# willi-menapace/PlayableEnvironments

Hardware: AMD Instinct MI355X
Metric: Mrays/s (higher is better)
Workload: dtype f32; 1 GPU; tennis renderer, 256x256 frame per GPU (rank r renders the frame of seed 1234 + r), 4 objects, 64+128 hierarchical samples/ray (coarse+fine networks), eval - BASELINE.json configs[1]; rays_per_gpu=65536, frames_per_gpu=1, parallelism=frame shard x1

## Files before the change

### include/playrender.h

```cpp
#ifndef PLAYRENDER_H
#define PLAYRENDER_H

#include <stddef.h>
#include <stdint.h>

#ifdef __cplusplus
extern "C" {
#endif

#define PR_ABI_VERSION 5
#define PR_MAX_OBJECTS 8
#define PR_MAX_LAYERS 12
#define PR_MAX_OCTAVES 16

typedef enum pr_status {
    PR_OK = 0,
    PR_ERR_INVALID = -1,
    PR_ERR_WORKSPACE = -2,
    PR_ERR_HIP = -3,
    PR_ERR_NO_DEVICE = -4
} pr_status;

#define PR_FLAG_PERTURB        1u
#define PR_FLAG_CANONICAL_POSE 2u
#define PR_FLAG_FIX_OVERLAPS   4u
#define PR_FLAG_NAIVE_MLP      8u
#define PR_FLAG_TRAIN_BN       16u

#define PR_FLAG_SAVE_FOR_BACKWARD 32u

#define PR_FLAG_GATE_HEAD 64u

#define PR_FLAG_DEVICE_NOISE 128u

#define PR_FLAG_SIGMOID_FEATURES 512u
#define PR_FLAG_SPLIT_BACKWARD 1024u
#define PR_FLAG_DIVERGENCE_GRAD 256u

typedef struct pr_linear_t {
    const float* weight;
    const float* bias;
    int32_t out_features;
    int32_t in_features;
} pr_linear_t;

typedef struct pr_object_model_t {
    int32_t kind;
    int32_t has_bender;
    int32_t positions;
    int32_t style_features;
    int32_t deformation_features;
    int32_t output_features;
    int32_t layers_width;
    int32_t backbone_count;
    int32_t skip_layer_idx;
    int32_t octaves;
    int32_t bender_width;
    int32_t bender_count;
    int32_t bender_skip;
// ... 246 lines not shown
```

### playableenvironments_amd/_lib.py

```python
from __future__ import annotations

import ctypes as C
import os
from typing import Optional

PR_MAX_OBJECTS = 8
PR_MAX_LAYERS = 12
PR_MAX_OCTAVES = 16

PR_FLAG_PERTURB = 1
PR_FLAG_CANONICAL_POSE = 2
PR_FLAG_FIX_OVERLAPS = 4
PR_FLAG_NAIVE_MLP = 8
PR_FLAG_TRAIN_BN = 16
PR_FLAG_SAVE_FOR_BACKWARD = 32
PR_FLAG_GATE_HEAD = 64
PR_FLAG_DEVICE_NOISE = 128
PR_FLAG_DIVERGENCE_GRAD = 256
PR_FLAG_SIGMOID_FEATURES = 512
PR_FLAG_SPLIT_BACKWARD = 1024
PR_PRECISION_FP32 = 0
PR_PRECISION_F16X3 = 1
PR_PRECISION_F16 = 2
PR_PROFILE_CATEGORIES = 8

c_float_p = C.POINTER(C.c_float)
c_int32_p = C.POINTER(C.c_int32)
c_uint8_p = C.POINTER(C.c_uint8)


class Linear(C.Structure):
    _fields_ = [("weight", C.c_void_p), ("bias", C.c_void_p), ("out_features", C.c_int32), ("in_features", C.c_int32)]


class ObjectModel(C.Structure):
    _fields_ = [
        ("kind", C.c_int32), ("has_bender", C.c_int32), ("positions", C.c_int32),
        ("style_features", C.c_int32), ("deformation_features", C.c_int32), ("output_features", C.c_int32),
        ("layers_width", C.c_int32), ("backbone_count", C.c_int32), ("skip_layer_idx", C.c_int32),
        ("octaves", C.c_int32), ("bender_width", C.c_int32), ("bender_count", C.c_int32),
        ("bender_skip", C.c_int32), ("bender_octaves", C.c_int32),
        ("bender_octave_weights", C.c_float * PR_MAX_OCTAVES),
        ("bbox", C.c_float * 6),
# ... 188 lines not shown
```

### playableenvironments_amd/csrc/backward.hip

```cpp
#include "pr_common.h"

#include <algorithm>
#include <map>
#include <utility>
#include <mutex>
#include "composite_dev.h"

namespace pr {

constexpr int BWD_SPLITS = 128;
constexpr int MAX_FCHUNK_B = 4;

struct CompositeBwdObject {
    const float* t;
    const float* sigma;
    const int32_t* slot;
    const float* dispmag;
    const float* feat;
    NoiseRef noise;
    int positions;
    pr_entry_grads_t g;
    float* g_feat;
    float* g_sigma;
    float* g_t;
    float* g_dm;
    const float* g_sample_t;
    const float* divergence;
    float* g_div;
// ... 1277 lines not shown
            gp.g_enc[k] = gtake(sizeof(float) * cap * encp);
            gp.gsr4[k] = gtake(sizeof(float) * cap * 4);
            gp.g_x[k] = gtake(sizeof(float) * cap * 3);
            gp.g_in6[k] = gtake(sizeof(float) * cap * 6);
            if (bc) {
                gp.g_braw4[k] = gtake(sizeof(float) * cap * 4);
                gp.bgstack[k] = gtake(sizeof(float) * cap * BWp * (size_t)bc);
                gp.g_benc[k] = gtake(sizeof(float) * cap * binp);
            }
        }
        gp.tn_partial_floats = tn_floats;
        gp.tn_partial = gtake(sizeof(float) * tn_floats);
        gp.zero_begin = goff;
        for (int k = 0; k < c.objects; ++k) {
            gp.sums[k] = gtake(sizeof(double) * 4 * MAX_WIDTH);
            gp.tables[k] = gtake(sizeof(float) * (size_t)c.frames * 4 * MAX_WIDTH);
        }
        gp.counters = gtake(sizeof(int32_t) * (4 * PR_MAX_OBJECTS + 8 * 4));
        gp.zero_bytes = goff - gp.zero_begin;
        gp.end = goff;
        gp.usable = !(c.flags & PR_FLAG_DIVERGENCE_GRAD) && (goff - lane_begin) <= GROUP_SCRATCH_LIMIT;
        if (gp.usable) bp->bytes = goff;
    }
    return PR_OK;
}

static int lane_stream(hipStream_t caller, hipStream_t* out) {
    static std::mutex mu;
    static std::map<std::pair<int, hipStream_t>, hipStream_t> streams;
    int dev = 0;
    PR_CHECK_HIP(hipGetDevice(&dev));
    std::lock_guard<std::mutex> lock(mu);
    hipStream_t& slot = streams[std::make_pair(dev, caller)];
    if (!slot) PR_CHECK_HIP(hipStreamCreateWithFlags(&slot, hipStreamNonBlocking));
    *out = slot;
    return PR_OK;
}

static int stream_wait(hipStream_t waiter, hipStream_t on) {
    constexpr int RING = 8;
    struct Ring { hipEvent_t e[RING] = {}; int next = 0; };
    static thread_local std::map<int, Ring> rings;
    int dev = 0;
    PR_CHECK_HIP(hipGetDevice(&dev));
    Ring& ring = rings[dev];
    hipEvent_t& e = ring.e[ring.next];
    ring.next = (ring.next + 1) % RING;
    if (!e) PR_CHECK_HIP(hipEventCreateWithFlags(&e, hipEventDisableTiming));
    PR_CHECK_HIP(hipEventRecord(e, on));
    PR_CHECK_HIP(hipStreamWaitEvent(waiter, e, 0));
    return PR_OK;
}

struct GemmCtx {
    const int32_t* rows;
    int max_rows;
    float* partial;
    hipStream_t s;
    float* gstack;
    float* chain_packed;
    size_t cap;
    const float* dw_acts;
    size_t dw_stride;
    const float* dw_in0;
};

static int weight_grad(const GemmCtx& g, const float* dY, int ldy, int n_out, const float* X, int ldx, int n_in, float* dW,
                       int ldw, float* dbias) {
    if (!dW && !dbias) return PR_OK;
    GemmTN p;
    memset(&p, 0, sizeof(p));
    p.A = dY; p.lda = ldy; p.B = X; p.ldb = ldx;
    p.rows = g.rows; p.ni = n_out; p.nj = n_in; p.splits = BWD_SPLITS;
// ... 928 lines not shown
```

### playableenvironments_amd/csrc/composite.hip

```cpp
#include "pr_common.h"
#include "composite_dev.h"

namespace pr {

struct CompositeSmem {
    float* tt;
    float* sg;
    float* dm;
    float* wo;
    float* wg;
    float* al;
    float* dv;
    int* sl;
    unsigned int* key;
};

constexpr int MAX_FCHUNK = 4;

__device__ __forceinline__ void transmittance_weights(float* al, int n, int lane) {
    float carry = 1.0f;
    for (int base = 0; base < n; base += 64) {
        const int j = base + lane;
        const float a = (j < n) ? al[j] : 0.f;
        float incl = (j < n) ? __fadd_rn(__fsub_rn(1.0f, a), 1e-10f) : 1.0f;
#pragma unroll
        for (int d = 1; d < 64; d <<= 1) {
            const float o = __shfl_up(incl, d, 64);
            if (lane >= d) incl *= o;
        }
        float excl = __shfl_up(incl, 1, 64);
        if (lane == 0) excl = 1.0f;
        if (j < n) al[j] = a * (carry * excl);
        carry *= __shfl(incl, 63, 64);
    }
}

constexpr int ROWS_IN_FLIGHT = 8;

__device__ __forceinline__ float sigmoid_of(float x) { return 1.0f / (1.0f + expf(-x)); }

template <int CW>
__device__ __forceinline__ void transmittance_weights_block(float* al, int n, float* totals, int wave, int lane) {
    if (CW == 1) {
        transmittance_weights(al, n, lane);
        return;
    }
    const int seg = (((n + CW - 1) / CW) + 63) & ~63;
    const int begin = wave * seg;
    const int end = (begin + seg < n) ? begin + seg : n;
    float carry = 1.0f;
    for (int base = begin; base < end; base += 64) {
        const int j = base + lane;
        const float a = (j < end) ? al[j] : 0.f;
        float incl = (j < end) ? __fadd_rn(__fsub_rn(1.0f, a), 1e-10f) : 1.0f;
#pragma unroll
        for (int d = 1; d < 64; d <<= 1) {
            const float o = __shfl_up(incl, d, 64);
            if (lane >= d) incl *= o;
        }
        float excl = __shfl_up(incl, 1, 64);
// ... 2 lines not shown
        carry *= __shfl(incl, 63, 64);
    }
    if (lane == 0) totals[wave] = carry;
    __syncthreads();
    float before = 1.0f;
    for (int w = 0; w < wave; ++w) before *= totals[w];
    if (wave > 0)
        for (int j = begin + lane; j < end; j += 64) al[j] *= before;
    __syncthreads();
}

template <int CW>
__device__ __forceinline__ float block_sum(float v, float* scratch, int wave, int lane) {
    v = wave_sum(v);
    if (CW == 1) return v;
    __syncthreads();
    if (lane == 0) scratch[wave] = v;
    __syncthreads();
    float total = 0.f;
    for (int w = 0; w < CW; ++w) total += scratch[w];
    return total;
}

template <int CW>
__global__ __launch_bounds__(64 * CW) void k_composite(CompositeParams p) {
    extern __shared__ __attribute__((aligned(16))) char raw_smem[];
    constexpr int CT = 64 * CW;
    const int S = p.sort_size;
    CompositeSmem sm;
    const int A = (p.total_positions + 63) & ~63;
    sm.key = reinterpret_cast<unsigned int*>(raw_smem);
    sm.tt = reinterpret_cast<float*>(sm.key + S);
    sm.sg = sm.tt + A;
    sm.dm = sm.sg + A;
    sm.wo = sm.dm + A;
    sm.wg = sm.sg;
    sm.al = sm.wo + A;
    const bool use_div = p.any_divergence != 0;
    sm.dv = use_div ? sm.al + A : nullptr;
    sm.sl = reinterpret_cast<int*>(sm.al + (use_div ? 2 * A : A));
    float* scratch = reinterpret_cast<float*>(sm.sl + A);
    unsigned long long* wide = p.fix_overlaps ? reinterpret_cast<unsigned long long*>(scratch + 4 * 64) : nullptr;

    const int tid = threadIdx.x, lane = tid & 63;
    const int wave = (CW == 1) ? 0 : __builtin_amdgcn_readfirstlane(tid >> 6);
    const long g = blockIdx.x;
    const float* d = p.ray_directions + (size_t)g * 3;
    const float norm = sqrtf(__fadd_rn(__fadd_rn(__fmul_rn(d[0], d[0]), __fmul_rn(d[1], d[1])), __fmul_rn(d[2], d[2])));
    const int PT = p.total_positions;

    {
        int off = 0;
        for (int k = 0; k < p.objects; ++k) {
            const CompositeObject& o = p.obj[k];
            const int P = o.positions;
            const size_t base = (size_t)g * P;
            for (int i = tid; i < P; i += CT) {
                sm.tt[off + i] = o.t[base + i];
                sm.sg[off + i] = o.sigma[base + i];
                sm.sl[off + i] = o.slot[base + i];
                sm.dm[off + i] = o.dispmag ? o.dispmag[base + i] : 0.f;
// ... 164 lines not shown
                w2 = sm.wg[off + i];
                take = row >= 0 && (w1 != 0.f || w2 != 0.f);
                if (p.sigmoid && row < 0) {
                    bare1 += w1;
                    bare2 += w2;
                }
            }
            const unsigned long long m = __ballot(take);
            if (take) {
                const int pos = off + begin + count + __popcll(m & ((1ull << lane) - 1ull));
                lrow[pos] = row;
                lw1[pos] = w1;
                sm.al[pos] = w2;
            }
            count += __popcll(m);
        }
        const int* rows_w = lrow + off + begin;
        const float* w1_w = lw1 + off + begin;
        const float* w2_w = sm.al + off + begin;
        float acco[MAX_FCHUNK];
#pragma unroll
        for (int c = 0; c < MAX_FCHUNK; ++c) acco[c] = 0.f;
        int i = 0;
        for (; i + ROWS_IN_FLIGHT <= count; i += ROWS_IN_FLIGHT) {
            float v[ROWS_IN_FLIGHT][MAX_FCHUNK];
#pragma unroll
            for (int u = 0; u < ROWS_IN_FLIGHT; ++u) {
                const float* f = o.feat + (size_t)rows_w[i + u] * F;
#pragma unroll
                for (int c = 0; c < MAX_FCHUNK; ++c) {
                    const int ch = lane + 64 * c;
                    v[u][c] = (ch < F) ? f[ch] : 0.f;
                    if (p.sigmoid) v[u][c] = sigmoid_of(v[u][c]);
                }
            }
#pragma unroll
            for (int u = 0; u < ROWS_IN_FLIGHT; ++u) {
                const float w1 = w1_w[i + u], w2 = w2_w[i + u];
#pragma unroll
                for (int c = 0; c < MAX_FCHUNK; ++c) {
                    acco[c] = __fadd_rn(acco[c], __fmul_rn(w1, v[u][c]));
                    accg[c] = __fadd_rn(accg[c], __fmul_rn(w2, v[u][c]));
                }
            }
        }
        for (; i < count; ++i) {
            const float* f = o.feat + (size_t)rows_w[i] * F;
            const float w1 = w1_w[i], w2 = w2_w[i];
#pragma unroll
            for (int c = 0; c < MAX_FCHUNK; ++c) {
                const int ch = lane + 64 * c;
                float v = (ch < F) ? f[ch] : 0.f;
                if (p.sigmoid) v = sigmoid_of(v);
                acco[c] = __fadd_rn(acco[c], __fmul_rn(w1, v));
                accg[c] = __fadd_rn(accg[c], __fmul_rn(w2, v));
            }
        }
        if (p.sigmoid) {
            bare1 = wave_sum(bare1);
            bare2 = wave_sum(bare2);
// ... 54 lines not shown
                scratch[wave * 64 + lane] = accg[c];
                __syncthreads();
                if (wave == 0)
                    for (int w = 1; w < CW; ++w) accg[c] = __fadd_rn(accg[c], scratch[w * 64 + lane]);
            }
        }
        if (wave == 0) {
            const int frame = (int)(g / p.rays);
            int r = (int)(g - (long)frame * p.rays);
            int grp = 0;
            while (grp < p.decoder.groups - 1 && r >= p.decoder.rays[grp]) r -= p.decoder.rays[grp++];
            const int c0 = p.decoder.channel_begin[grp], c1 = p.decoder.channel_end[grp];
            const size_t cells = (size_t)p.decoder.rays[grp];
            float* map = p.decoder.map[grp] + (size_t)frame * (c1 - c0) * cells + r;
#pragma unroll
            for (int c = 0; c < MAX_FCHUNK; ++c) {
                const int ch = lane + 64 * c;
                if (ch >= c0 && ch < c1 && ch < F) map[(size_t)(ch - c0) * cells] = accg[c];
            }
        }
    }
}

int launch_composite(const CompositeParams& p, hipStream_t s) {
    PR_REQUIRE(p.F <= 64 * MAX_FCHUNK, "output_features %d exceeds %d", p.F, 64 * MAX_FCHUNK);
    PR_REQUIRE(p.sort_size >= p.total_positions && (p.sort_size & (p.sort_size - 1)) == 0, "bad sort size");
    for (int k = 0; k < p.objects; ++k)
        PR_REQUIRE(p.obj[k].positions <= 64 * 32, "positions per ray %d too large for the overlap mask", p.obj[k].positions);
    const size_t lds = (size_t)p.sort_size * 4 + (size_t)((p.total_positions + 63) & ~63) * (p.any_divergence ? 7 : 6) * 4 +
                       sizeof(float) * 4 * 64 + (p.fix_overlaps ? (size_t)p.sort_size * 8 : 0);
    PR_REQUIRE(lds <= 156 * 1024, "too many samples per ray for the compositing kernel (%d)", p.total_positions);
    if (p.decoder.groups > 0) {
        PR_REQUIRE(p.decoder.groups <= PR_MAX_DECODER_GROUPS, "decoder layout: %d groups (max %d)", p.decoder.groups, PR_MAX_DECODER_GROUPS);
        long sum = 0;
        for (int i = 0; i < p.decoder.groups; ++i) {
            PR_REQUIRE(p.decoder.rays[i] > 0 && p.decoder.width[i] > 0 && p.decoder.rays[i] % p.decoder.width[i] == 0,
                       "decoder layout: group %d has %d rays in rows of %d", i, p.decoder.rays[i], p.decoder.width[i]);
            PR_REQUIRE(p.decoder.channel_begin[i] >= 0 && p.decoder.channel_begin[i] < p.decoder.channel_end[i] && p.decoder.channel_end[i] <= p.F,
                       "decoder layout: group %d channel range [%d, %d) outside 0..%d", i, p.decoder.channel_begin[i], p.decoder.channel_end[i], p.F);
            PR_REQUIRE(p.decoder.map[i] != nullptr, "decoder layout: group %d has no map", i);
            sum += p.decoder.rays[i];
        }
        PR_REQUIRE(sum == p.rays, "decoder layout: the groups hold %ld rays, the call has %d", sum, p.rays);
    }
    const long total = (long)p.frames * p.rays;
    ProfileScope scope(1, s);
    if (p.total_positions >= 256) {
        PR_TRY(prepare_kernel(reinterpret_cast<const void*>(&k_composite<4>), 156 * 1024, nullptr));
        hipLaunchKernelGGL(k_composite<4>, dim3((unsigned)total), dim3(256), lds, s, p);
    } else {
        PR_TRY(prepare_kernel(reinterpret_cast<const void*>(&k_composite<1>), 156 * 1024, nullptr));
        hipLaunchKernelGGL(k_composite<1>, dim3((unsigned)total), dim3(64), lds, s, p);
    }
    PR_LAUNCH_CHECK();
    return PR_OK;
}

}
```

### playableenvironments_amd/csrc/pr_common.h

```cpp
#pragma once

#include <hip/hip_runtime.h>
#include <stdint.h>
#include <stdio.h>
#include <string.h>

#include "playrender.h"

namespace pr {

void set_error(const char* fmt, ...);

#define PR_CHECK_HIP(expr)                                                              \
    do {                                                                                \
        hipError_t _e = (expr);                                                         \
        if (_e != hipSuccess) {                                                         \
            pr::set_error("%s failed: %s (%s:%d)", #expr, hipGetErrorString(_e), __FILE__, __LINE__); \
            return PR_ERR_HIP;                                                          \
        }                                                                               \
    } while (0)

#define PR_REQUIRE(cond, ...)                                                           \
    do {                                                                                \
        if (!(cond)) {                                                                  \
// ... 344 lines not shown
    const float* t;
    const float* sigma;
    const int32_t* slot;
    const float* divergence;
    const float* dispmag;
    const float* feat;
    NoiseRef noise;
    int positions;
    pr_entry_t out;
};
struct CompositeParams {
    int frames, rays, objects, static_objects, F;
    int fix_overlaps;
    int any_divergence;
    int sigmoid;
    int total_positions;
    int sort_size;
    const float* ray_directions;
    NoiseRef noise_global;
    CompositeObject obj[PR_MAX_OBJECTS];
    pr_entry_t global;
    pr_decoder_layout_t decoder;
};
int launch_composite(const CompositeParams& p, hipStream_t s);

#define PR_TRY(expr)                 \
    do {                             \
        int _r = (expr);             \
        if (_r != PR_OK) return _r;  \
    } while (0)

struct SavedPlan {
    size_t rec_pos, rec_flat, row_flags, enc, act, h1, h2, batch, stat_count, bin, bact, braw, delta, div, bits, bbits, stats;
};
struct TypePlan {
    size_t t[PR_MAX_OBJECTS], sigma[PR_MAX_OBJECTS], slot[PR_MAX_OBJECTS], dispmag[PR_MAX_OBJECTS];
    size_t adain[PR_MAX_OBJECTS];
    size_t feat[PR_MAX_OBJECTS];
    int positions[PR_MAX_OBJECTS];
    size_t totals;
    size_t head_counts;
    size_t zero_begin, zero_bytes;
    SavedPlan saved[PR_MAX_OBJECTS];
};
struct Plan {
    TypePlan type[2];
    size_t block_sums, block_offsets;
    size_t rec_pos, rec_flat;
    size_t pend_act, pend_meta;
    size_t h1, h2, row_flags, stats, stat_count, batch_stats;
    size_t div_t0, div_ta, div_tb;
    size_t rec_pos_k[PR_MAX_OBJECTS], rec_flat_k[PR_MAX_OBJECTS];
    size_t bytes;
    int nblocks256;
};
int prepare_kernel(const void* kernel, int lds_bytes, int* cu_count);
int launch_zero_fill(void* dst, size_t bytes, hipStream_t s);
int validate_call(const pr_call_t& c, const pr_object_t* objs);
bool group_active(const pr_call_t& c);
bool group_train_active(const pr_call_t& c);
bool gate_active(const pr_call_t& c);
bool group_active(const pr_call_t& c);
int make_plan(const pr_call_t& c, const pr_object_t* objs, Plan* plan);
void bbox_split(const pr_object_model_t& m, float* lo, float* hi, float* size);
int build_mlp_layers(const pr_object_model_t& m, const ModelDims& d, const PackedLayout& l, const float* base,
                     MlpParams* p, bool split3 = false);

struct GemmNN {
    const float* A; int lda;
    const float* B; int ldb;
    float* C; int ldc;
    const int32_t* rows;
    int n, k;
    int accumulate;
    const float* mask; int ldm;
    int b_transposed;
    int k_valid;
};
int launch_gemm_nn(const GemmNN& p, int max_rows, hipStream_t s);

struct GemmTN {
    const float* A; int lda;
    const float* B; int ldb;
    float* C; int ldc;
// ... 84 lines not shown
    int32_t* counters;
    int split_precision;
};
size_t tn_all_partial_floats(int ni, int nj, long max_rows);
int launch_gemm_tn_all(TnAll& g, const long* max_rows, hipStream_t s);

struct DivergenceParams {
    const int32_t* total; int max_rows;
    const int32_t* rec_flat; const int32_t* row_flags; const float* rec_pos;
    NoiseRef noise;
    int positions;
    const float* bin; int bin_pad, benc, b_octaves;
    const float* bacts; size_t bact_stride; int BW, BWpad, b_count, b_skip, bin_real;
    const pr_linear_t* layers; pr_linear_t out_head;
    const float* braw;
    float lo[3], hi[3];
    int canonical;
    float* t0; float* ta; float* tb;
    float* tstack; size_t tstride;
    float* div;
};
int launch_divergence(const DivergenceParams& p, hipStream_t s);

struct ProfileScope {
    ProfileScope(int category, hipStream_t s);
    ~ProfileScope();
    int category_;
    hipStream_t stream_;
    hipEvent_t start_;
    bool active_;
};

#ifdef __HIPCC__
__device__ __forceinline__ void philox4x32_10(unsigned int c0, unsigned int c1, unsigned int c2, unsigned int c3, unsigned int k0,
                                              unsigned int k1, unsigned int* out) {
#pragma unroll
    for (int round = 0; round < 10; ++round) {
        const unsigned int hi0 = __umulhi(0xD2511F53u, c0), lo0 = 0xD2511F53u * c0;
        const unsigned int hi1 = __umulhi(0xCD9E8D57u, c2), lo1 = 0xCD9E8D57u * c2;
        const unsigned int n0 = hi1 ^ c1 ^ k0, n2 = hi0 ^ c3 ^ k1;
        c0 = n0; c1 = lo1; c2 = n2; c3 = lo0;
        k0 += 0x9E3779B9u;
        k1 += 0xBB67AE85u;
    }
    out[0] = c0; out[1] = c1; out[2] = c2; out[3] = c3;
}
// ... 74 lines not shown
```

### playableenvironments_amd/csrc/render.hip

```cpp
#include "pr_common.h"

#include <stdarg.h>

#include <atomic>
#include <mutex>
#include <vector>

namespace pr {

struct ProfileRecord { int category; hipEvent_t start, stop; };
static std::atomic<bool> g_profile_on{false};
static std::vector<ProfileRecord> g_profile;
static std::mutex g_profile_mutex;

int prepare_kernel(const void* kernel, int lds_bytes, int* cu_count) {
    struct Entry { const void* kernel; int device; int cus; };
    static std::vector<Entry> done;
    static std::mutex guard;
    int dev = 0;
    PR_CHECK_HIP(hipGetDevice(&dev));
    std::lock_guard<std::mutex> lock(guard);
    for (const Entry& e : done)
        if (e.kernel == kernel && e.device == dev) {
            if (cu_count) *cu_count = e.cus;
            return PR_OK;
        }
    PR_CHECK_HIP(hipFuncSetAttribute(kernel, hipFuncAttributeMaxDynamicSharedMemorySize, lds_bytes));
    hipDeviceProp_t prop;
// ... 37 lines not shown
    if (!active_) return;
    hipEvent_t stop;
    if (hipEventCreate(&stop) != hipSuccess) return;
    if (hipEventRecord(stop, stream_) != hipSuccess) {
        (void)hipEventDestroy(stop);
        (void)hipEventDestroy(start_);
        return;
    }
    std::lock_guard<std::mutex> lock(g_profile_mutex);
    g_profile.push_back(ProfileRecord{category_, start_, stop});
}

static thread_local char g_error[512] = "";

void set_error(const char* fmt, ...) {
    va_list ap;
    va_start(ap, fmt);
    vsnprintf(g_error, sizeof(g_error), fmt, ap);
    va_end(ap);
}

int build_mlp_layers(const pr_object_model_t& m, const ModelDims& d, const PackedLayout& l, const float* base,
                     MlpParams* p, bool split3);

static size_t align_up(size_t v) { return (v + 255) & ~(size_t)255; }

int validate_call(const pr_call_t& c, const pr_object_t* objs) {
    PR_REQUIRE(c.frames > 0 && c.rays > 0, "empty call: %d frames x %d rays", c.frames, c.rays);
    PR_REQUIRE(c.objects >= 1 && c.objects <= PR_MAX_OBJECTS, "objects %d out of range 1..%d", c.objects, PR_MAX_OBJECTS);
    PR_REQUIRE(c.static_objects >= 0 && c.static_objects <= c.objects, "static_objects %d out of range", c.static_objects);
    PR_REQUIRE((long)c.frames * c.rays < (1L << 31), "too many rays in one call");
    PR_REQUIRE(c.ray_origins && c.ray_directions && c.w2o && c.style && c.deformation && c.object_in_scene,
               "NULL input pointer");
    PR_REQUIRE(c.precision == PR_PRECISION_FP32 || c.precision == PR_PRECISION_F16X3 || c.precision == PR_PRECISION_F16,
               "unknown precision %d", c.precision);
    PR_REQUIRE(!(c.precision != PR_PRECISION_FP32 && (c.flags & PR_FLAG_TRAIN_BN)),
               "the fp16 kernels have no train-mode BatchNorm phases: use PR_PRECISION_FP32 for training");
    PR_REQUIRE(!(c.precision != PR_PRECISION_FP32 && (c.flags & PR_FLAG_SAVE_FOR_BACKWARD)),
               "differentiable calls run on the exact kernel: use PR_PRECISION_FP32 with PR_FLAG_SAVE_FOR_BACKWARD");
    PR_REQUIRE(!(c.flags & PR_FLAG_SAVE_FOR_BACKWARD) || !(c.flags & PR_FLAG_NAIVE_MLP), "the scalar debugging kernel saves nothing");
    for (int k = 0; k < c.objects; ++k) {
        const pr_object_model_t& m = objs[k].coarse;
        PR_REQUIRE(m.positions >= 1, "object %d: positions_count_coarse %d", k, m.positions);
        PR_REQUIRE(c.linspace_coarse[k] != nullptr, "object %d: linspace_coarse missing", k);
        PR_REQUIRE(objs[k].packed_coarse != nullptr, "object %d: packed coarse weights missing", k);
        PR_REQUIRE((long)c.frames * c.rays * (long)m.positions < (1L << 31), "too many samples in one call");
// ... 120 lines not shown
    if (div_t) {
        plan->div_t0 = take(sizeof(float) * div_t0);
        plan->div_ta = take(sizeof(float) * div_t);
        plan->div_tb = take(sizeof(float) * div_t);
    }
    if (c.flags & PR_FLAG_SAVE_FOR_BACKWARD) {
        for (int t = 0; t < ntypes; ++t) {
            const size_t arena = take(feat_bytes[t]);
            for (int k = 0; k < c.objects; ++k) plan->type[t].feat[k] += arena;
        }
    } else {
        const size_t arena = take(feat_bytes[0] > feat_bytes[1] ? feat_bytes[0] : feat_bytes[1]);
        for (int t = 0; t < ntypes; ++t)
            for (int k = 0; k < c.objects; ++k) plan->type[t].feat[k] += arena;
    }
    plan->bytes = off;
    return PR_OK;
}

bool group_active(const pr_call_t& c) {
    return !(c.flags & (PR_FLAG_TRAIN_BN | PR_FLAG_SAVE_FOR_BACKWARD | PR_FLAG_NAIVE_MLP)) && c.objects > 1;
}

bool group_train_active(const pr_call_t& c) {
    return (c.flags & PR_FLAG_SAVE_FOR_BACKWARD) && !(c.flags & PR_FLAG_NAIVE_MLP) && c.objects > 1;
}

void bbox_split(const pr_object_model_t& m, float* lo, float* hi, float* size) {
    for (int a = 0; a < 3; ++a) {
        lo[a] = m.bbox[2 * a];
        hi[a] = m.bbox[2 * a + 1];
        if (size) size[a] = m.bbox[2 * a + 1] - m.bbox[2 * a];
    }
}

static int render(const pr_call_t& c, const pr_object_t* objs, const pr_outputs_t* outs[2], char* ws, const Plan& plan,
                  hipStream_t s) {
    const int ntypes = c.use_fine ? 2 : 1;
    const int K = c.objects;
    int32_t* block_sums_all = reinterpret_cast<int32_t*>(ws + plan.block_sums);
    int32_t* block_offsets_all = reinterpret_cast<int32_t*>(ws + plan.block_offsets);
    const bool place_grouped = c.objects > 1 && ((c.flags & PR_FLAG_SAVE_FOR_BACKWARD) || group_active(c));
    static thread_local PlaceParams place_jobs[PR_MAX_OBJECTS];
    static thread_local FillParams fill_jobs[PR_MAX_OBJECTS];
    int32_t* total_ptrs[PR_MAX_OBJECTS];
    float* rec_pos = reinterpret_cast<float*>(ws + plan.rec_pos);
    int32_t* rec_flat = reinterpret_cast<int32_t*>(ws + plan.rec_flat);
    const bool naive = (c.flags & PR_FLAG_NAIVE_MLP) != 0;
    const bool gate = gate_active(c);
    const bool grouped = group_active(c);
    MlpParams jobs[PR_MAX_OBJECTS];
    int job_rows[PR_MAX_OBJECTS];
    FoldParams fold_jobs[PR_MAX_OBJECTS];
    const bool train_grouped = group_train_active(c);
    struct TrainJob {
        MlpParams mp; FoldParams fo; ModelDims d; const pr_object_model_t* m; const SavedPlan* sv;
        double* stats; int32_t* stat_count; float* batch; float* h1; float* h2; float* rec_pos; int32_t* rec_flat;
        int k, P, max_tiles; bool frozen, save;
    };
    static thread_local TrainJob train_jobs[PR_MAX_OBJECTS];
// ... 294 lines not shown
                DivChainJob& q = dj[div_jobs];
                memset(&q, 0, sizeof(q));
                q.total = totals + k; q.rec_flat = J.rec_flat; q.row_flags = J.mp.row_flags; q.rec_pos = J.rec_pos;
                q.noise = probes; q.positions = J.P;
                q.bin = J.mp.save_bin; q.bin_pad = J.d.bin_pad; q.benc = J.d.benc; q.b_octaves = m.bender_octaves;
                q.bbits = J.mp.save_bbits; q.bbits_stride = J.mp.save_bbits_stride;
                q.BW = J.d.BW; q.BWpad = J.d.BWpad; q.b_count = m.bender_count; q.b_skip = m.bender_skip;
                for (int j = 0; j < m.bender_count; ++j) q.seg0[j] = Seg{packed + l.b_seg_off[j][0], (j == 0 ? J.d.bin_pad : J.d.BWpad) / 8, 0};
                q.seg1 = Seg{packed + l.b_seg_off[m.bender_skip][1], J.d.bin_pad / 8, 0};
                q.w_out = packed + l.b_out_off;
                q.braw = J.mp.save_braw;
                bbox_split(m, q.lo, q.hi, nullptr);
                q.canonical = (c.flags & PR_FLAG_CANONICAL_POSE) ? 1 : 0;
                q.div = reinterpret_cast<float*>(ws + J.sv->div);
                q.tile_counter = head_counts + 2 * PR_MAX_OBJECTS + k;
                div_rows[div_jobs] = (long)cap_rows;
                ++div_jobs;
            }
            if (div_jobs) PR_TRY(launch_div_chain_group(dj, div_rows, div_jobs, s));
        }

        if (grouped) {
            PR_TRY(launch_adain_fold_group(fold_jobs, K, s));
            if (c.precision != PR_PRECISION_FP32)
                PR_TRY(launch_mlp_split_group(jobs, job_rows, K, c.precision == PR_PRECISION_F16 ? 1 : 3, s));
            else
                PR_TRY(launch_mlp_group(jobs, job_rows, K, s));
        }

        const pr_outputs_t* out = outs[t];
        CompositeParams cp;
        memset(&cp, 0, sizeof(cp));
        cp.frames = c.frames; cp.rays = c.rays; cp.objects = K; cp.static_objects = c.static_objects;
        cp.F = objs[0].coarse.output_features;
        cp.fix_overlaps = (c.flags & PR_FLAG_FIX_OVERLAPS) ? 1 : 0;
        cp.sigmoid = (c.flags & PR_FLAG_SIGMOID_FEATURES) ? 1 : 0;
        cp.total_positions = total_positions;
        int ss = 64;
        while (ss < total_positions) ss <<= 1;
        cp.sort_size = ss;
        cp.ray_directions = c.ray_directions;
        cp.noise_global = perturb_noise(noise.integrate_global, c, NOISE_INTEGRATE_GLOBAL, t, 0);
        for (int k = 0; k < K; ++k) {
            const pr_object_model_t& m = t ? objs[k].fine : objs[k].coarse;
            PR_REQUIRE(m.output_features == cp.F, "all objects must share output_features");
            CompositeObject& o = cp.obj[k];
            o.t = reinterpret_cast<const float*>(ws + tp.t[k]);
            o.sigma = reinterpret_cast<const float*>(ws + tp.sigma[k]);
            o.slot = reinterpret_cast<const int32_t*>(ws + tp.slot[k]);
            o.dispmag = m.has_bender ? reinterpret_cast<const float*>(ws + tp.dispmag[k]) : nullptr;
            o.divergence = ((c.flags & PR_FLAG_SAVE_FOR_BACKWARD) && m.has_bender)
                               ? reinterpret_cast<const float*>(ws + tp.saved[k].div) : nullptr;
            if (o.divergence) cp.any_divergence = 1;
            o.feat = reinterpret_cast<const float*>(ws + tp.feat[k]);
            o.noise = perturb_noise(noise.integrate[k], c, NOISE_INTEGRATE, t, k);
            o.positions = m.positions;
            if (out) o.out = out->object[k];
        }
        if (out) {
            cp.global = out->global;
            cp.decoder = out->decoder;
        }
        PR_TRY(launch_composite(cp, s));

        if (out) {
            for (int k = 0; k < K; ++k) {
                const size_t cap = (size_t)c.frames * c.rays * tp.positions[k];
                if (out->sample_t[k])
                    PR_CHECK_HIP(hipMemcpyAsync(out->sample_t[k], ws + tp.t[k], sizeof(float) * cap, hipMemcpyDeviceToDevice, s));
                if (out->sample_sigma[k])
                    PR_CHECK_HIP(hipMemcpyAsync(out->sample_sigma[k], ws + tp.sigma[k], sizeof(float) * cap, hipMemcpyDeviceToDevice, s));
                if (out->sample_slot[k])
                    PR_CHECK_HIP(hipMemcpyAsync(out->sample_slot[k], ws + tp.slot[k], sizeof(int32_t) * cap, hipMemcpyDeviceToDevice, s));
            }
            if (out->evaluated_samples)
                PR_CHECK_HIP(hipMemcpyAsync(out->evaluated_samples, totals, sizeof(int32_t) * K, hipMemcpyDeviceToDevice, s));
            if (out->head_samples)
                PR_CHECK_HIP(hipMemcpyAsync(out->head_samples, gate ? head_counts : totals, sizeof(int32_t) * K,
                                            hipMemcpyDeviceToDevice, s));
        }
    }
    return PR_OK;
}

}

extern "C" int pr_workspace_size(const pr_call_t* call, const pr_object_t* objects, size_t* bytes) {
    PR_REQUIRE(call && objects && bytes, "pr_workspace_size: NULL argument");
    PR_TRY(pr::validate_call(*call, objects));
    pr::Plan plan;
    PR_TRY(pr::make_plan(*call, objects, &plan));
    *bytes = plan.bytes;
    return PR_OK;
}

extern "C" int pr_render_forward(const pr_call_t* call, const pr_object_t* objects, const pr_outputs_t* coarse,
                                 const pr_outputs_t* fine, void* workspace, size_t workspace_bytes, void* stream) {
    PR_REQUIRE(call && objects && workspace, "pr_render_forward: NULL argument");
    PR_TRY(pr::validate_call(*call, objects));
    pr::Plan plan;
    PR_TRY(pr::make_plan(*call, objects, &plan));
    if (workspace_bytes < plan.bytes) {
        pr::set_error("workspace too small: %zu bytes given, %zu needed", workspace_bytes, plan.bytes);
        return PR_ERR_WORKSPACE;
    }
// ... 112 lines not shown
```

### playableenvironments_amd/environment_model.py

```python
from __future__ import annotations

import collections.abc
import ctypes as C
import math
import warnings
from typing import Dict, List, Tuple

import torch
import torch.nn as nn

from . import _lib, ray_sampling
from .modules import REGISTRATION_EPOCH as _REGISTRATION_EPOCH, CameraParametersStorage, ModuleList, Tracked
from .object_composer import ObjectComposer, ObjectIDsHelper


def euler_to_matrix(rotations: torch.Tensor, translations: torch.Tensor) -> torch.Tensor:
    cx, sx = torch.cos(rotations[..., 0]), torch.sin(rotations[..., 0])
    cy, sy = torch.cos(rotations[..., 1]), torch.sin(rotations[..., 1])
    cz, sz = torch.cos(rotations[..., 2]), torch.sin(rotations[..., 2])
    zero, one = torch.zeros_like(cx), torch.ones_like(cx)
    rx = torch.stack([one, zero, zero, zero, cx, -sx, zero, sx, cx], -1).reshape(cx.shape + (3, 3))
    ry = torch.stack([cy, zero, sy, zero, one, zero, -sy, zero, cy], -1).reshape(cx.shape + (3, 3))
    rz = torch.stack([cz, -sz, zero, sz, cz, zero, zero, zero, one], -1).reshape(cx.shape + (3, 3))
    rot = torch.matmul(ry, torch.matmul(rx, rz))
# ... 667 lines not shown

    def __getstate__(self):
        state = dict(self.__dict__)
        state.update(_replays={}, _in_replay=False, _pixel_cache={}, _edge_point_cache={}, _axes_point_cache={})
        return state

    def _replay_signature(self, name: str):
        composer = self.object_composer
        owner = None if name == "scene_encodings" else self
        params = composer._parameter_list(owner)
        root = composer if owner is None else self
        if composer._tree_is_tracked(root):
            tree = _REGISTRATION_EPOCH[0]
        else:
            tree = tuple(b.data_ptr() for b in root.buffers())
        decoder = None
        if self.use_image_decoder and name == "scene_encodings":
            decoder = tuple(t.data_ptr() for m in (self.image_decoder, self.grid_sampler) if isinstance(m, nn.Module)
                            for t in list(m.parameters()) + list(m.buffers()))
        return (tuple((p.data_ptr(), p._version) for p in params), tree, decoder, composer.precision, bool(composer.gate_feature_head),
                composer.state_epoch, composer.weights_epoch,
                None if composer.object_entry_fields is None else tuple(composer.object_entry_fields),
                bool(self.fused_scene_setup), bool(composer.training), bool(composer.use_naive_mlp), float(self.focal_length_multiplier),
                int(composer.max_workspace_bytes))

    def _replayed(self, name: str, method, tensors, statics: tuple):
        from .frame_graph import CapturedCall
        key = (name, tuple((tuple(t.shape), t.dtype, str(t.device)) for t in tensors), statics)
        signature = self._replay_signature(name)
        entry = self._replays.get(key)
        if entry is not None and entry[0] != signature:
            del self._replays[key]
            entry = None
        if entry is None:
            while len(self._replays) >= max(1, int(self.frame_replay_slots)):
                self._replays.pop(next(iter(self._replays)))
            self._replays[key] = (signature, None)
            return None
        if entry[1] is None:
            self._in_replay = True
            try:
                recorded = CapturedCall(lambda *ts: method(*ts), list(tensors), warmup=1, what=f"frame_replay ({name})")
            except Exception as error:
                torch.cuda.synchronize()
                warnings.warn(f"frame_replay: recording the {name} evaluation call failed ({type(error).__name__}: {error}); calls of "
                              "this shape run eagerly from now on", RuntimeWarning)
                recorded = False
# ... 501 lines not shown
```

### playableenvironments_amd/frame_graph.py

```python
from __future__ import annotations

import contextlib
import gc
import os
from typing import Dict, Tuple

import torch

SCENE_KEYS = ("camera_rotations", "camera_translations", "focals", "object_rotation_parameters",
              "object_translation_parameters", "object_style", "object_deformation", "object_in_scene")

GRAPH_RUNTIME_SWITCH = ("DEBUG_CLR_GRAPH_PACKET_CAPTURE", "0")


@contextlib.contextmanager
def _no_collections_while_recording():
    gc.collect()
    was_enabled = gc.isenabled()
    gc.disable()
    try:
        yield
    finally:
        if was_enabled:
            gc.enable()
# ... 75 lines not shown
            self._weights_version = self._signature()
            self.graph = torch.cuda.CUDAGraph(keep_graph=True)
            try:
                with _no_collections_while_recording(), torch.cuda.graph(self.graph), torch.no_grad():
                    self.results = self._call()
            except BaseException:
                import traceback
                traceback.print_exc()
                raise
            self.census = _checked_recording(self.graph, f"FrameGraph(mode={mode!r})")
            self.graph.instantiate()
        finally:
            model._in_replay = was_recording
        self._packed = [entry[1] for entry in composer._packed.values()]
        self._linspace = list(composer._linspace.values())
        if composer._workspace is not self._workspace:
            raise RuntimeError("the composer re-allocated its workspace during the capture")

    def _signature(self):
        composer = self.model.object_composer
        owner = composer if self.mode == "scene_encodings" else self.model
        return (tuple((p.data_ptr(), p._version) for p in owner.parameters()), composer.precision,
                bool(composer.gate_feature_head), composer.state_epoch, composer.weights_epoch,
                None if composer.object_entry_fields is None else tuple(composer.object_entry_fields))

    def render(self, scene: Dict[str, torch.Tensor]) -> Dict:
        if self._signature() != self._weights_version:
            raise RuntimeError("the composer's parameters, precision or annealing step changed since the frame was captured: "
                               "build a new FrameGraph")
        for k in self.keys:
            src = scene[k]
            if src.shape != self.inputs[k].shape:
                raise ValueError(f"{k}: shape {tuple(src.shape)} differs from the captured {tuple(self.inputs[k].shape)}")
            self.inputs[k].copy_(src, non_blocking=True)
        self.graph.replay()
        return self.results


class CapturedCall:

    def __init__(self, fn, tensors, warmup: int = 2, what: str = "CapturedCall"):
        self.inputs = [t.detach().clone() for t in tensors]
        device = self.inputs[0].device
        side = torch.cuda.Stream(device)
        side.wait_stream(torch.cuda.current_stream(device))
        with torch.cuda.stream(side), torch.no_grad():
            for _ in range(max(1, warmup)):
# ... 55 lines not shown
```

### playableenvironments_amd/object_composer.py

```python
from __future__ import annotations

import ctypes as C
import math
import threading
import warnings
import weakref
from typing import Dict, List, Optional, Tuple

import torch
import torch.nn as nn

from . import _lib
from .modules import OBJECT_MODEL_CLASSES, REGISTRATION_EPOCH as _REGISTRATION_EPOCH, ModuleList, RayBendingStyleNerfModel, Tracked, \
    tree_is_tracked


ENTRY_KEYS = ("integrated_features", "opacity", "weights", "depth", "disparity",
              "integrated_displacements_magnitude", "integrated_divergence")

_AWAITING_STEP: "weakref.WeakSet" = weakref.WeakSet()
_AWAITING_LOCK = threading.Lock()
_STEP_HOOK = []


# ... 324 lines not shown
        self.object_models_coarse = ModuleList(self.create_object_models(fine=False))
        self.object_models_fine = ModuleList(self.create_object_models(fine=True))
        self.apply_activation = self.config["model"]["apply_activation"]
        if self.object_models_coarse[0].model_config["nerf_model"]["output_features"] != 3 and self.apply_activation:
            raise Exception("The application of activations to the nerf output is requested, but the model seem not "
                            "to output colors directly. Please make sure this is the behavior you desire")
        self.object_id_helper = ObjectIDsHelper(self.config)
        self.state_epoch = 0
        self.weights_epoch = 0
        self._packed: Dict[tuple, tuple] = {}
        self._param_lists: Dict[int, list] = {}
        self._structs: Dict[tuple, tuple] = {}
        self._tracked: Dict[int, bool] = {}
        self._registration_epoch = _REGISTRATION_EPOCH[0]
        self._budget_ok = 0
        self._annealing: Dict[int, tuple] = {}
        self._host_step: Optional[int] = 0
        self._linspace: Dict[tuple, torch.Tensor] = {}
        self._workspace: Optional[torch.Tensor] = None
        self.use_naive_mlp = False
        self.precision = "fp32"
        self._noted_split_training = False
        self.gate_feature_head = True
        self.last_normalised_samples: Dict[str, torch.Tensor] = {}
        self.noise_source = "device"
        self.noise_seed_source = "host"
        self.last_noise_seed = None
        self.batchnorm_check = "eager"
        self._pending_bn_check: Optional[tuple] = None
        self.object_entry_fields: Optional[Tuple[str, ...]] = None
        self.gradient_hooks: List = []

    def _raise_pending_batchnorm_check(self):
        if torch.cuda.is_current_stream_capturing():
            return
        pending, self._pending_bn_check = self._pending_bn_check, None
        if pending is None:
            return
        host, event, types, count = pending
        event.synchronize()
        counts = host.tolist()
        for i, ty in enumerate(types):
            cur = counts[i * count:(i + 1) * count]
            if any(c == 1 for c in cur):
                raise ValueError(f"Expected more than 1 value per channel when training, got {cur} evaluated "
                                 f"samples per object ({ty} pass of the previous composer call)")
# ... 426 lines not shown
            flags |= _lib.PR_FLAG_PERTURB
        if canonical_pose:
            flags |= _lib.PR_FLAG_CANONICAL_POSE
        if self.config["model"]["fix_object_overlaps"] and _object_ids is None:
            flags |= _lib.PR_FLAG_FIX_OVERLAPS
        if self.apply_activation:
            flags |= _lib.PR_FLAG_SIGMOID_FEATURES
        if self.use_naive_mlp:
            flags |= _lib.PR_FLAG_NAIVE_MLP
        if self.training:
            flags |= _lib.PR_FLAG_TRAIN_BN
        if _save:
            flags |= _lib.PR_FLAG_SAVE_FOR_BACKWARD
            if self.precision in ("f16x3", "f16"):
                flags |= _lib.PR_FLAG_SPLIT_BACKWARD
                if not self._noted_split_training:
                    self._noted_split_training = True
                    warnings.warn(f"ObjectComposer.precision = {self.precision!r} applies to this differentiable call too: phase 1 of the "
                                  "forward pass, the backward chains and the weight gradients run on fp16 pairs of power-of-two scaled operands "
                                  "(fp32 accumulation; gradients within the fp32 path's tolerances).  Set precision = 'fp32' for exact-fp32 "
                                  "training.", UserWarning, stacklevel=2)
        if self.gate_feature_head:
            flags |= _lib.PR_FLAG_GATE_HEAD

        types = ["coarse"] + (["fine"] if use_fine else [])
        object_fields = None
        if self.object_entry_fields is not None and not _save and not self.training:
            object_fields = tuple(self.object_entry_fields)
            unknown = [f for f in object_fields if f not in ENTRY_KEYS]
            if unknown:
                raise ValueError(f"object_entry_fields: unknown field(s) {unknown}; the fields are {ENTRY_KEYS}")
        ptot = {"coarse": pc, "fine": [a + b for a, b in zip(pc, pf)]}
        noise: Dict[str, torch.Tensor] = {}
        if self.noise_source not in ("device", "torch"):
            raise ValueError(f"unknown noise_source {self.noise_source!r} (expected 'device' or 'torch')")
        needs_noise = perturb or (_save and self.training)
        device_noise = needs_noise and _noise is None and self.noise_source == "device"
        noise_seed = 0
        seed_word = None
        capturing = torch.cuda.is_current_stream_capturing()
        if device_noise:
            flags |= _lib.PR_FLAG_DEVICE_NOISE
            if self.noise_seed_source not in ("host", "device"):
                raise ValueError(f"unknown noise_seed_source {self.noise_seed_source!r} (expected 'host' or 'device')")
            if self.noise_seed_source == "device" or capturing:
                seed_word = torch.randint(0, 2 ** 62, (1,), dtype=torch.int64, device=dev)
# ... 340 lines not shown
```

Baseline: 0.3219 Mrays/s.

## Overlap coarse compositing with fine-pass work on an auxiliary stream

During inference with the fine network and grouped MLPs, the coarse-pass compositing kernel and its output copies are forked onto a per-caller auxiliary stream. The main stream then continues with fine-pass sampling and setup, and joins the auxiliary stream just before the grouped fine MLP launch and again at the end of the call. The forked compositing runs a slim kernel variant with fewer rows in flight and a high waves-per-EU hint so it can share the GPU with concurrent kernels. The lane-stream helper moves into render.hip with bounded LRU eviction, and a serial-schedule flag is added to turn the overlap off. The extra event waits add some host overhead, and the gain depends on whether the composite and the fine-pass kernels actually run concurrently.

```diff
diff --git a/include/playrender.h b/include/playrender.h
--- a/include/playrender.h
+++ b/include/playrender.h
@@ -35,6 +35,7 @@
 
 #define PR_FLAG_SIGMOID_FEATURES 512u
 #define PR_FLAG_SPLIT_BACKWARD 1024u
+#define PR_FLAG_SERIAL_SCHEDULE 2048u
 #define PR_FLAG_DIVERGENCE_GRAD 256u
 
 typedef struct pr_linear_t {
diff --git a/playableenvironments_amd/_lib.py b/playableenvironments_amd/_lib.py
--- a/playableenvironments_amd/_lib.py
+++ b/playableenvironments_amd/_lib.py
@@ -19,6 +19,7 @@
 PR_FLAG_DIVERGENCE_GRAD = 256
 PR_FLAG_SIGMOID_FEATURES = 512
 PR_FLAG_SPLIT_BACKWARD = 1024
+PR_FLAG_SERIAL_SCHEDULE = 2048
 PR_PRECISION_FP32 = 0
 PR_PRECISION_F16X3 = 1
 PR_PRECISION_F16 = 2
diff --git a/playableenvironments_amd/csrc/backward.hip b/playableenvironments_amd/csrc/backward.hip
--- a/playableenvironments_amd/csrc/backward.hip
+++ b/playableenvironments_amd/csrc/backward.hip
@@ -1,9 +1,6 @@
 #include "pr_common.h"
 
 #include <algorithm>
-#include <map>
-#include <utility>
-#include <mutex>
 #include "composite_dev.h"
 
 namespace pr {
@@ -1327,33 +1324,6 @@
         gp.usable = !(c.flags & PR_FLAG_DIVERGENCE_GRAD) && (goff - lane_begin) <= GROUP_SCRATCH_LIMIT;
         if (gp.usable) bp->bytes = goff;
     }
-    return PR_OK;
-}
-
-static int lane_stream(hipStream_t caller, hipStream_t* out) {
-    static std::mutex mu;
-    static std::map<std::pair<int, hipStream_t>, hipStream_t> streams;
-    int dev = 0;
-    PR_CHECK_HIP(hipGetDevice(&dev));
-    std::lock_guard<std::mutex> lock(mu);
-    hipStream_t& slot = streams[std::make_pair(dev, caller)];
-    if (!slot) PR_CHECK_HIP(hipStreamCreateWithFlags(&slot, hipStreamNonBlocking));
-    *out = slot;
-    return PR_OK;
-}
-
-static int stream_wait(hipStream_t waiter, hipStream_t on) {
-    constexpr int RING = 8;
-    struct Ring { hipEvent_t e[RING] = {}; int next = 0; };
-    static thread_local std::map<int, Ring> rings;
-    int dev = 0;
-    PR_CHECK_HIP(hipGetDevice(&dev));
-    Ring& ring = rings[dev];
-    hipEvent_t& e = ring.e[ring.next];
-    ring.next = (ring.next + 1) % RING;
-    if (!e) PR_CHECK_HIP(hipEventCreateWithFlags(&e, hipEventDisableTiming));
-    PR_CHECK_HIP(hipEventRecord(e, on));
-    PR_CHECK_HIP(hipStreamWaitEvent(waiter, e, 0));
     return PR_OK;
 }
 
diff --git a/playableenvironments_amd/csrc/composite.hip b/playableenvironments_amd/csrc/composite.hip
--- a/playableenvironments_amd/csrc/composite.hip
+++ b/playableenvironments_amd/csrc/composite.hip
@@ -36,6 +36,7 @@
 }
 
 constexpr int ROWS_IN_FLIGHT = 8;
+constexpr int ROWS_IN_FLIGHT_SLIM = 4;
 
 __device__ __forceinline__ float sigmoid_of(float x) { return 1.0f / (1.0f + expf(-x)); }
 
@@ -84,8 +85,10 @@
     return total;
 }
 
-template <int CW>
-__global__ __launch_bounds__(64 * CW) void k_composite(CompositeParams p) {
+template <int CW, bool SLIM>
+__global__ __launch_bounds__(64 * CW) __attribute__((amdgpu_waves_per_eu(SLIM ? 8 : 1)))
+void k_composite(CompositeParams p) {
+    constexpr int RIF = SLIM ? ROWS_IN_FLIGHT_SLIM : ROWS_IN_FLIGHT;
     extern __shared__ __attribute__((aligned(16))) char raw_smem[];
     constexpr int CT = 64 * CW;
     const int S = p.sort_size;
@@ -98,7 +101,7 @@
     sm.wo = sm.dm + A;
     sm.wg = sm.sg;
     sm.al = sm.wo + A;
-    const bool use_div = p.any_divergence != 0;
+    const bool use_div = !SLIM && p.any_divergence != 0;
     sm.dv = use_div ? sm.al + A : nullptr;
     sm.sl = reinterpret_cast<int*>(sm.al + (use_div ? 2 * A : A));
     float* scratch = reinterpret_cast<float*>(sm.sl + A);
@@ -309,10 +312,10 @@
 #pragma unroll
         for (int c = 0; c < MAX_FCHUNK; ++c) acco[c] = 0.f;
         int i = 0;
-        for (; i + ROWS_IN_FLIGHT <= count; i += ROWS_IN_FLIGHT) {
-            float v[ROWS_IN_FLIGHT][MAX_FCHUNK];
-#pragma unroll
-            for (int u = 0; u < ROWS_IN_FLIGHT; ++u) {
+        for (; i + RIF <= count; i += RIF) {
+            float v[RIF][MAX_FCHUNK];
+#pragma unroll
+            for (int u = 0; u < RIF; ++u) {
                 const float* f = o.feat + (size_t)rows_w[i + u] * F;
 #pragma unroll
                 for (int c = 0; c < MAX_FCHUNK; ++c) {
@@ -322,7 +325,7 @@
                 }
             }
 #pragma unroll
-            for (int u = 0; u < ROWS_IN_FLIGHT; ++u) {
+            for (int u = 0; u < RIF; ++u) {
                 const float w1 = w1_w[i + u], w2 = w2_w[i + u];
 #pragma unroll
                 for (int c = 0; c < MAX_FCHUNK; ++c) {
@@ -423,7 +426,7 @@
     }
 }
 
-int launch_composite(const CompositeParams& p, hipStream_t s) {
+int launch_composite(const CompositeParams& p, hipStream_t s, bool slim) {
     PR_REQUIRE(p.F <= 64 * MAX_FCHUNK, "output_features %d exceeds %d", p.F, 64 * MAX_FCHUNK);
     PR_REQUIRE(p.sort_size >= p.total_positions && (p.sort_size & (p.sort_size - 1)) == 0, "bad sort size");
     for (int k = 0; k < p.objects; ++k)
@@ -446,13 +449,12 @@
     }
     const long total = (long)p.frames * p.rays;
     ProfileScope scope(1, s);
-    if (p.total_positions >= 256) {
-        PR_TRY(prepare_kernel(reinterpret_cast<const void*>(&k_composite<4>), 156 * 1024, nullptr));
-        hipLaunchKernelGGL(k_composite<4>, dim3((unsigned)total), dim3(256), lds, s, p);
-    } else {
-        PR_TRY(prepare_kernel(reinterpret_cast<const void*>(&k_composite<1>), 156 * 1024, nullptr));
-        hipLaunchKernelGGL(k_composite<1>, dim3((unsigned)total), dim3(64), lds, s, p);
-    }
+    const bool wide = p.total_positions >= 256;
+    PR_REQUIRE(!(slim && p.any_divergence), "the slim compositing kernel has no divergence column");
+    void (*kernel)(CompositeParams) = wide ? (slim ? &k_composite<4, true> : &k_composite<4, false>)
+                                           : (slim ? &k_composite<1, true> : &k_composite<1, false>);
+    PR_TRY(prepare_kernel(reinterpret_cast<const void*>(kernel), 156 * 1024, nullptr));
+    hipLaunchKernelGGL(kernel, dim3((unsigned)total), dim3(wide ? 256 : 64), lds, s, p);
     PR_LAUNCH_CHECK();
     return PR_OK;
 }
diff --git a/playableenvironments_amd/csrc/pr_common.h b/playableenvironments_amd/csrc/pr_common.h
--- a/playableenvironments_amd/csrc/pr_common.h
+++ b/playableenvironments_amd/csrc/pr_common.h
@@ -390,7 +390,7 @@
     pr_entry_t global;
     pr_decoder_layout_t decoder;
 };
-int launch_composite(const CompositeParams& p, hipStream_t s);
+int launch_composite(const CompositeParams& p, hipStream_t s, bool slim = false);
 
 #define PR_TRY(expr)                 \
     do {                             \
@@ -428,6 +428,7 @@
 bool group_active(const pr_call_t& c);
 bool group_train_active(const pr_call_t& c);
 bool gate_active(const pr_call_t& c);
+bool overlap_active(const pr_call_t& c);
 bool group_active(const pr_call_t& c);
 int make_plan(const pr_call_t& c, const pr_object_t* objs, Plan* plan);
 void bbox_split(const pr_object_model_t& m, float* lo, float* hi, float* size);
@@ -558,6 +559,9 @@
 };
 int launch_divergence(const DivergenceParams& p, hipStream_t s);
 
+int lane_stream(hipStream_t caller, hipStream_t* out);
+int stream_wait(hipStream_t waiter, hipStream_t on);
+
 struct ProfileScope {
     ProfileScope(int category, hipStream_t s);
     ~ProfileScope();
diff --git a/playableenvironments_amd/csrc/render.hip b/playableenvironments_amd/csrc/render.hip
--- a/playableenvironments_amd/csrc/render.hip
+++ b/playableenvironments_amd/csrc/render.hip
@@ -3,7 +3,9 @@
 #include <stdarg.h>
 
 #include <atomic>
+#include <map>
 #include <mutex>
+#include <utility>
 #include <vector>
 
 namespace pr {
@@ -87,6 +89,70 @@
 
 int build_mlp_layers(const pr_object_model_t& m, const ModelDims& d, const PackedLayout& l, const float* base,
                      MlpParams* p, bool split3);
+
+constexpr size_t LANE_STREAMS = 32;
+
+int lane_stream(hipStream_t caller, hipStream_t* out) {
+    struct Lane { hipStream_t stream; unsigned long long used; };
+    static std::mutex mu;
+    static std::map<std::pair<int, hipStream_t>, Lane> lanes;
+    static unsigned long long clock = 0;
+    int dev = 0;
+    PR_CHECK_HIP(hipGetDevice(&dev));
+    std::lock_guard<std::mutex> lock(mu);
+    const auto key = std::make_pair(dev, caller);
+    auto it = lanes.find(key);
+    if (it == lanes.end()) {
+        hipStreamCaptureStatus capturing = hipStreamCaptureStatusNone;
+        if (lanes.size() >= LANE_STREAMS && hipStreamIsCapturing(caller, &capturing) == hipSuccess &&
+            capturing == hipStreamCaptureStatusNone) {
+            auto victim = lanes.end();
+            for (auto l = lanes.begin(); l != lanes.end(); ++l) {
+                if (l->first.first != dev || (victim != lanes.end() && l->second.used >= victim->second.used)) continue;
+                hipStreamCaptureStatus st = hipStreamCaptureStatusNone;
+                if (hipStreamIsCapturing(l->second.stream, &st) != hipSuccess || st != hipStreamCaptureStatusNone) continue;
+                if (hipStreamQuery(l->second.stream) != hipSuccess) {
+                    (void)hipGetLastError();
+                    continue;
+                }
+                victim = l;
+            }
+            if (victim != lanes.end()) {
+                (void)hipStreamDestroy(victim->second.stream);
+                lanes.erase(victim);
+            }
+        }
+        hipStream_t created = nullptr;
+        PR_CHECK_HIP(hipStreamCreateWithFlags(&created, hipStreamNonBlocking));
+        it = lanes.emplace(key, Lane{created, 0}).first;
+    }
+    it->second.used = ++clock;
+    *out = it->second.stream;
+    return PR_OK;
+}
+
+int stream_wait(hipStream_t waiter, hipStream_t on) {
+    constexpr int RING = 8;
+    struct Ring { hipEvent_t e[RING] = {}; int next = 0; };
+    struct Rings {
+        std::map<int, Ring> of_device;
+        ~Rings() {
+            for (auto& r : of_device)
+                for (hipEvent_t e : r.second.e)
+                    if (e) (void)hipEventDestroy(e);
+        }
+    };
+    static thread_local Rings rings;
+    int dev = 0;
+    PR_CHECK_HIP(hipGetDevice(&dev));
+    Ring& ring = rings.of_device[dev];
+    hipEvent_t& e = ring.e[ring.next];
+    ring.next = (ring.next + 1) % RING;
+    if (!e) PR_CHECK_HIP(hipEventCreateWithFlags(&e, hipEventDisableTiming));
+    PR_CHECK_HIP(hipEventRecord(e, on));
+    PR_CHECK_HIP(hipStreamWaitEvent(waiter, e, 0));
+    return PR_OK;
+}
 
 static size_t align_up(size_t v) { return (v + 255) & ~(size_t)255; }
 
@@ -253,6 +319,10 @@
     return !(c.flags & (PR_FLAG_TRAIN_BN | PR_FLAG_SAVE_FOR_BACKWARD | PR_FLAG_NAIVE_MLP)) && c.objects > 1;
 }
 
+bool overlap_active(const pr_call_t& c) {
+    return c.use_fine && group_active(c) && !(c.flags & PR_FLAG_SERIAL_SCHEDULE);
+}
+
 bool group_train_active(const pr_call_t& c) {
     return (c.flags & PR_FLAG_SAVE_FOR_BACKWARD) && !(c.flags & PR_FLAG_NAIVE_MLP) && c.objects > 1;
 }
@@ -265,8 +335,8 @@
     }
 }
 
-static int render(const pr_call_t& c, const pr_object_t* objs, const pr_outputs_t* outs[2], char* ws, const Plan& plan,
-                  hipStream_t s) {
+static int enqueue_call(const pr_call_t& c, const pr_object_t* objs, const pr_outputs_t* outs[2], char* ws, const Plan& plan,
+                        hipStream_t s, hipStream_t aux, bool* open_fork) {
     const int ntypes = c.use_fine ? 2 : 1;
     const int K = c.objects;
     int32_t* block_sums_all = reinterpret_cast<int32_t*>(ws + plan.block_sums);
@@ -607,12 +677,22 @@
 
         if (grouped) {
             PR_TRY(launch_adain_fold_group(fold_jobs, K, s));
+            if (*open_fork) {
+                PR_TRY(stream_wait(s, aux));
+                *open_fork = false;
+            }
             if (c.precision != PR_PRECISION_FP32)
                 PR_TRY(launch_mlp_split_group(jobs, job_rows, K, c.precision == PR_PRECISION_F16 ? 1 : 3, s));
             else
                 PR_TRY(launch_mlp_group(jobs, job_rows, K, s));
         }
 
+        hipStream_t cs = s;
+        if (aux && t == 0) {
+            PR_TRY(stream_wait(aux, s));
+            *open_fork = true;
+            cs = aux;
+        }
         const pr_outputs_t* out = outs[t];
         CompositeParams cp;
         memset(&cp, 0, sizeof(cp));
@@ -646,26 +726,37 @@
             cp.global = out->global;
             cp.decoder = out->decoder;
         }
-        PR_TRY(launch_composite(cp, s));
+        PR_TRY(launch_composite(cp, cs, cs != s));
 
         if (out) {
             for (int k = 0; k < K; ++k) {
                 const size_t cap = (size_t)c.frames * c.rays * tp.positions[k];
                 if (out->sample_t[k])
-                    PR_CHECK_HIP(hipMemcpyAsync(out->sample_t[k], ws + tp.t[k], sizeof(float) * cap, hipMemcpyDeviceToDevice, s));
+                    PR_CHECK_HIP(hipMemcpyAsync(out->sample_t[k], ws + tp.t[k], sizeof(float) * cap, hipMemcpyDeviceToDevice, cs));
                 if (out->sample_sigma[k])
-                    PR_CHECK_HIP(hipMemcpyAsync(out->sample_sigma[k], ws + tp.sigma[k], sizeof(float) * cap, hipMemcpyDeviceToDevice, s));
+                    PR_CHECK_HIP(hipMemcpyAsync(out->sample_sigma[k], ws + tp.sigma[k], sizeof(float) * cap, hipMemcpyDeviceToDevice, cs));
                 if (out->sample_slot[k])
-                    PR_CHECK_HIP(hipMemcpyAsync(out->sample_slot[k], ws + tp.slot[k], sizeof(int32_t) * cap, hipMemcpyDeviceToDevice, s));
+                    PR_CHECK_HIP(hipMemcpyAsync(out->sample_slot[k], ws + tp.slot[k], sizeof(int32_t) * cap, hipMemcpyDeviceToDevice, cs));
             }
             if (out->evaluated_samples)
-                PR_CHECK_HIP(hipMemcpyAsync(out->evaluated_samples, totals, sizeof(int32_t) * K, hipMemcpyDeviceToDevice, s));
+                PR_CHECK_HIP(hipMemcpyAsync(out->evaluated_samples, totals, sizeof(int32_t) * K, hipMemcpyDeviceToDevice, cs));
             if (out->head_samples)
                 PR_CHECK_HIP(hipMemcpyAsync(out->head_samples, gate ? head_counts : totals, sizeof(int32_t) * K,
-                                            hipMemcpyDeviceToDevice, s));
-        }
-    }
-    return PR_OK;
+                                            hipMemcpyDeviceToDevice, cs));
+        }
+    }
+    return PR_OK;
+}
+
+static int render(const pr_call_t& c, const pr_object_t* objs, const pr_outputs_t* outs[2], char* ws, const Plan& plan,
+                  hipStream_t s) {
+    hipStream_t aux = nullptr;
+    if (overlap_active(c)) PR_TRY(lane_stream(s, &aux));
+    bool open_fork = false;
+    const int status = enqueue_call(c, objs, outs, ws, plan, s, aux, &open_fork);
+    if (!open_fork) return status;
+    const int joined = stream_wait(s, aux);
+    return status != PR_OK ? status : joined;
 }
 
 }
diff --git a/playableenvironments_amd/environment_model.py b/playableenvironments_amd/environment_model.py
--- a/playableenvironments_amd/environment_model.py
+++ b/playableenvironments_amd/environment_model.py
@@ -713,7 +713,7 @@
                 composer.state_epoch, composer.weights_epoch,
                 None if composer.object_entry_fields is None else tuple(composer.object_entry_fields),
                 bool(self.fused_scene_setup), bool(composer.training), bool(composer.use_naive_mlp), float(self.focal_length_multiplier),
-                int(composer.max_workspace_bytes))
+                int(composer.max_workspace_bytes), bool(composer.serial_schedule))
 
     def _replayed(self, name: str, method, tensors, statics: tuple):
         from .frame_graph import CapturedCall
diff --git a/playableenvironments_amd/frame_graph.py b/playableenvironments_amd/frame_graph.py
--- a/playableenvironments_amd/frame_graph.py
+++ b/playableenvironments_amd/frame_graph.py
@@ -121,7 +121,7 @@
         owner = composer if self.mode == "scene_encodings" else self.model
         return (tuple((p.data_ptr(), p._version) for p in owner.parameters()), composer.precision,
                 bool(composer.gate_feature_head), composer.state_epoch, composer.weights_epoch,
-                None if composer.object_entry_fields is None else tuple(composer.object_entry_fields))
+                None if composer.object_entry_fields is None else tuple(composer.object_entry_fields), bool(composer.serial_schedule))
 
     def render(self, scene: Dict[str, torch.Tensor]) -> Dict:
         if self._signature() != self._weights_version:
diff --git a/playableenvironments_amd/object_composer.py b/playableenvironments_amd/object_composer.py
--- a/playableenvironments_amd/object_composer.py
+++ b/playableenvironments_amd/object_composer.py
@@ -370,6 +370,7 @@
         self.precision = "fp32"
         self._noted_split_training = False
         self.gate_feature_head = True
+        self.serial_schedule = False
         self.last_normalised_samples: Dict[str, torch.Tensor] = {}
         self.noise_source = "device"
         self.noise_seed_source = "host"
@@ -842,6 +843,8 @@
                                   "training.", UserWarning, stacklevel=2)
         if self.gate_feature_head:
             flags |= _lib.PR_FLAG_GATE_HEAD
+        if self.serial_schedule:
+            flags |= _lib.PR_FLAG_SERIAL_SCHEDULE
 
         types = ["coarse"] + (["fine"] if use_fine else [])
         object_fields = None
```

Result: no change. 0.3233 Mrays/s (median of 6 runs) (+0.4%).
